# eigenkernel/eigenkernel

Hardware: AMD Instinct MI355X
Metric: eigenpairs/s (full spectrum) + achieved fp64 TFLOP/s vs roofline, N=16384 GEP (higher is better)
Workload: dtype f64

## Files before the change

eigenkernel_amd/csrc/ek_chol.hip:

```cpp
#include "ek_common.h"
#include "ek_block64.h"

#include <cstdlib>
#include <vector>

namespace ek {
namespace {

constexpr int NB = kDiagNB;
constexpr size_t kDiagLds = 2 * b64::IMG * sizeof(double);

__global__ __launch_bounds__(256) void potrf_diag_kernel(int nb, double *B, int ldb, double *inv, int *info,
                                                         int info_base) {
  using namespace b64;
  extern __shared__ double smem[];
  double *sP = smem, *sQ = smem + IMG;
  __shared__ double s_scr[kScratch];
  const int t = threadIdx.x, lane = t & 63, wave = t >> 6, l15 = lane & 15, l4 = lane >> 4;
  auto upper = [&](int gr, int gc) -> double {
    if (gc < nb) return B[(size_t)gc + (size_t)gr * ldb];
    return (gr == gc) ? 1.0 : 0.0;
  };
  auto fail_exit = [&](int j) {
    if (t == 0) atomicCAS(info, 0, info_base + j + 1);
    for (int idx = t; idx < NB * NB; idx += 256)
      inv[idx] = ((idx & (NB - 1)) == (idx >> 7)) ? 1.0 : 0.0;
  };
  for (int idx = t; idx < SB * SB; idx += 256) {
    const int c = idx & 63, r = idx >> 6;
    sP[r * LD + c] = (c >= r) ? upper(r, c) : 0.0;
  }
  __syncthreads();
  int fail = chol64_upper_wg(sP, s_scr);
  if (fail >= 0) { fail_exit(fail); return; }
// ... 197 lines not shown
                 double *work) {
  set_attrs();
  if (n <= 0) return;
  potrf_rec(s, n, B, ldb, 0, invdiag, d_info, work);
}

void trtri256_blocks(hipStream_t s, int n, const double *L, int ldl, const double *invdiag, double *inv256, double *scratch) {
  const int nb2 = n / (2 * NB);
  if (nb2 <= 0) return;
  GemmDesc g{};
  g.M = NB; g.N = NB; g.K = NB; g.transA = false; g.transB = false; g.alpha = 1.0; g.beta = 0.0; g.batch = nb2; g.lower_only = false;
  g.A = L + NB; g.lda = ldl; g.strideA = (long long)2 * NB * ((long long)ldl + 1);
  g.B = invdiag; g.ldb = NB; g.strideB = (long long)2 * NB * NB;
  g.C = scratch; g.ldc = NB; g.strideC = (long long)NB * NB;
  gemm(s, g);
  g.alpha = -1.0;
  g.A = invdiag + (size_t)NB * NB; g.lda = NB; g.strideA = (long long)2 * NB * NB;
  g.B = scratch; g.ldb = NB; g.strideB = (long long)NB * NB;
  g.C = inv256 + NB; g.ldc = 2 * NB; g.strideC = (long long)4 * NB * NB;
  gemm(s, g);
  hipLaunchKernelGGL(inv256_assemble_kernel, dim3(nb2), dim3(256), 0, s, invdiag, inv256);
}
void trsm_register_inv256(const double *invdiag, const double *inv256, int n) {
  g_inv256.base128 = inv256 ? invdiag : nullptr; g_inv256.inv256 = inv256; g_inv256.nblk256 = inv256 ? n / (2 * NB) : 0;
}

void trtri_diag_blocks(hipStream_t s, int n, const double *L, int ldl, double *invdiag) {
  set_attrs();
  if (n <= 0) return;
  hipLaunchKernelGGL(trtri_diag_kernel, dim3(ceil_div(n, NB)), dim3(256),
                     (NB * NB + NB) * sizeof(double), s, n, L, ldl, invdiag);
}


void trsm_rlt(hipStream_t s, int m, int n, const double *L, int ldl, const double *invdiag,
              double *X, int ldx, double *work) {
  if (m <= 0 || n <= 0) return;
  if (const double *i2 = leaf256(invdiag, n)) {
    gemm(s, false, true, m, n, n, 1.0, X, ldx, i2, 2 * NB, 0.0, work, m);
    copy_matrix(s, m, n, work, m, X, ldx);
    return;
  }
  if (n <= NB) {
    gemm(s, false, true, m, n, n, 1.0, X, ldx, invdiag, NB, 0.0, work, m);
    copy_matrix(s, m, n, work, m, X, ldx);
    return;
  }
  const int n1 = split_t(n), n2 = n - n1;
  double *X2 = X + (size_t)n1 * ldx;
  const double *L21 = L + n1, *L22 = L + (size_t)n1 + (size_t)n1 * ldl;
  trsm_rlt(s, m, n1, L, ldl, invdiag, X, ldx, work);
  gemm(s, false, true, m, n2, n1, -1.0, X, ldx, L21, ldl, 1.0, X2, ldx);
  trsm_rlt(s, m, n2, L22, ldl, invdiag + (size_t)(n1 / NB) * NB * NB, X2, ldx, work);
}

void trsm_lln(hipStream_t s, int n, int m, const double *L, int ldl, const double *invdiag,
              double *X, int ldx, double *work) {
  if (m <= 0 || n <= 0) return;
  if (const double *i2 = leaf256(invdiag, n)) {
    gemm(s, false, false, n, m, n, 1.0, i2, 2 * NB, X, ldx, 0.0, work, n);
    copy_matrix(s, n, m, work, n, X, ldx);
    return;
  }
  if (n <= NB) {
    gemm(s, false, false, n, m, n, 1.0, invdiag, NB, X, ldx, 0.0, work, n);
    copy_matrix(s, n, m, work, n, X, ldx);
    return;
  }
  const int n1 = split_t(n), n2 = n - n1;
  double *X2 = X + n1;
  const double *L21 = L + n1, *L22 = L + (size_t)n1 + (size_t)n1 * ldl;
  trsm_lln(s, n1, m, L, ldl, invdiag, X, ldx, work);
  gemm(s, false, false, n2, m, n1, -1.0, L21, ldl, X, ldx, 1.0, X2, ldx);
  trsm_lln(s, n2, m, L22, ldl, invdiag + (size_t)(n1 / NB) * NB * NB, X2, ldx, work);
}

void trsm_llt(hipStream_t s, int n, int m, const double *L, int ldl, const double *invdiag,
              double *X, int ldx, double *work) {
  if (m <= 0 || n <= 0) return;
  if (const double *i2 = leaf256(invdiag, n)) {
    gemm(s, true, false, n, m, n, 1.0, i2, 2 * NB, X, ldx, 0.0, work, n);
    copy_matrix(s, n, m, work, n, X, ldx);
    return;
  }
  if (n <= NB) {
    gemm(s, true, false, n, m, n, 1.0, invdiag, NB, X, ldx, 0.0, work, n);
    copy_matrix(s, n, m, work, n, X, ldx);
    return;
  }
  const int n1 = split_t(n), n2 = n - n1;
  double *X2 = X + n1;
  const double *L21 = L + n1, *L22 = L + (size_t)n1 + (size_t)n1 * ldl;
  trsm_llt(s, n2, m, L22, ldl, invdiag + (size_t)(n1 / NB) * NB * NB, X2, ldx, work);
  gemm(s, true, false, n1, m, n2, -1.0, L21, ldl, X2, ldx, 1.0, X, ldx);
  trsm_llt(s, n1, m, L, ldl, invdiag, X, ldx, work);
}

__global__ void axpy_matrix_kernel(int m, int n, double alpha, const double *__restrict__ src, int lds,
                                   double *__restrict__ dst, int ldd) {
  const int i = blockIdx.x * blockDim.x + threadIdx.x;
  if (i >= m) return;
  for (int j = blockIdx.y; j < n; j += gridDim.y)
    dst[(size_t)i + (size_t)j * ldd] += alpha * src[(size_t)i + (size_t)j * lds];
}
__global__ void full_from_lower_kernel(int n, const double *__restrict__ src, int lds,
                                       double *__restrict__ dst, int ldd) {
  const int i = blockIdx.x * blockDim.x + threadIdx.x;
  if (i >= n) return;
  for (int j = blockIdx.y; j < n; j += gridDim.y)
    dst[(size_t)i + (size_t)j * ldd] = (i >= j) ? src[(size_t)i + (size_t)j * lds] : src[(size_t)j + (size_t)i * lds];
}
__global__ __launch_bounds__(256) void syr2k_fold_kernel(int n, const double *__restrict__ M, int ldm,
                                                         double *__restrict__ A, int lda) {
  __shared__ double sT[32][33];
  const int bi = blockIdx.x, bj = blockIdx.y;
  if (bj > bi) return;
  const int tx = threadIdx.x & 31, ty = threadIdx.x >> 5;
#pragma unroll
  for (int q = 0; q < 4; ++q) {
    const int r = 32 * bj + tx, c = 32 * bi + ty + 8 * q;
// ... 394 lines not shown

void potrf_lower_rl(hipStream_t s, hipStream_t s2, int n, double *B, int ldb, double *invdiag, int *d_info,
                    void *work) {
  set_attrs();
  if (n <= 0) return;
  const PotrfDistLayout Ly(n, ldb, 1);
  const int NRB = Ly.NRB;
  char *w = (char *)work;
  double *ppan = (double *)(w + Ly.off_pbuf);
  int *infos = (int *)(w + Ly.off_infos);
  double *infod = (double *)(w + Ly.off_infod);
  long long *offs = (long long *)(w + Ly.off_offs);
  int *dims = (int *)(w + Ly.off_dims);
  static hipEvent_t evU[2], evP[2], evFork;
  static bool ev_ready = false;
  if (!ev_ready) {
    for (int i = 0; i < 2; ++i) {
      (void)hipEventCreateWithFlags(&evU[i], hipEventDisableTiming);
      (void)hipEventCreateWithFlags(&evP[i], hipEventDisableTiming);
    }
    (void)hipEventCreateWithFlags(&evFork, hipEventDisableTiming);
    ev_ready = true;
  }
  (void)hipMemsetAsync(infos, 0, (size_t)NRB * sizeof(int), s);
  hipLaunchKernelGGL(potrf_table_kernel, dim3(NRB), dim3(round_up(Ly.maxb, 64)), 0, s, n, ldb, 1, 0, NRB, Ly.maxb,
                     offs, dims);
  auto factor_panel = [&](hipStream_t st, int k) {
    const int off = k * NB, nbk = (n - off < NB) ? n - off : NB, mrows = n - off - nbk;
    double *Bd = B + (size_t)off + (size_t)off * ldb;
    double *inv = invdiag + (size_t)k * NB * NB;
    hipLaunchKernelGGL(potrf_diag_kernel, dim3(1), dim3(256), kDiagLds, st, nbk, Bd,
                       ldb, inv, infos + k, off);
    if (mrows > 0) {
      gemm(st, false, true, mrows, nbk, nbk, 1.0, Bd + nbk, ldb, inv, NB, 0.0, ppan, mrows);
      copy_matrix(st, mrows, nbk, ppan, mrows, Bd + nbk, ldb);
    }
  };
  constexpr int ob = 4;
  const int NOB = ceil_div(NRB, ob);
  auto factor_outer = [&](hipStream_t st, int o) {
    const int k0 = o * ob, k1 = (k0 + ob < NRB) ? k0 + ob : NRB;
    for (int k = k0; k < k1; ++k) {
      factor_panel(st, k);
      const int cnt = k1 - 1 - k;
      if (cnt > 0) {
        const int nbk = (n - k * NB < NB) ? n - k * NB : NB;
        GemmDesc g{};
        g.N = NB; g.K = nbk; g.transA = false; g.transB = true; g.alpha = -1.0; g.beta = 1.0;
        g.A = B; g.lda = ldb; g.B = B; g.ldb = ldb; g.C = B; g.ldc = ldb; g.lower_only = true;
        g.even_offs = true;
        g.M = n - (k + 1) * NB; g.batch = cnt;
        g.d_offs = offs + (size_t)k * Ly.maxb * 3; g.d_dims = dims + (size_t)k * Ly.maxb * 3;
        gemm(st, g);
      }
    }
  };
  (void)hipEventRecord(evFork, s);
  (void)hipStreamWaitEvent(s2, evFork, 0);
  factor_outer(s2, 0);
  (void)hipEventRecord(evP[0], s2);
  for (int o = 0; o + 1 < NOB; ++o) {
    const int c0 = o * ob * NB, c1 = (o + 1) * ob * NB, kw = c1 - c0;
    const int m2 = n - c1;
    const int wnext = (m2 < ob * NB) ? m2 : ob * NB;
    (void)hipStreamWaitEvent(s, evP[o & 1], 0);
    const double *P = B + (size_t)c1 + (size_t)c0 * ldb;
    double *C = B + (size_t)c1 + (size_t)c1 * ldb;
    gemm(s, false, true, m2, wnext, kw, -1.0, P, ldb, P, ldb, 1.0, C, ldb, true);
// ... 60 lines not shown
```

eigenkernel_amd/csrc/ek_common.h:

```cpp
#pragma once
#include <hip/hip_runtime.h>
#include <cstddef>
#include <cstdint>
#include <cstdio>

#define EK_HIP_CHECK(expr)                                                              \
  do {                                                                                  \
    hipError_t _e = (expr);                                                             \
    if (_e != hipSuccess) {                                                             \
      fprintf(stderr, "[ek_hip] %s failed at %s:%d: %s\n", #expr, __FILE__, __LINE__,   \
              hipGetErrorString(_e));                                                   \
      return -1000 - (int)_e;                                                           \
    }                                                                                   \
  } while (0)

namespace ek {

constexpr int kWave = 64;

inline int ceil_div(int a, int b) { return (a + b - 1) / b; }
inline int round_up(int a, int b) { return ceil_div(a, b) * b; }

struct GemmDesc {
  int M, N, K;
// ... 43 lines not shown
void set_matrix(hipStream_t s, int m, int n, double offdiag, double diag, double *A, int lda);
void symmetrize_lower(hipStream_t s, int n, double *A, int lda);
void transpose_rows(hipStream_t s, int n, int m, const double *src, int lds, int r0, double *dst, int ldd);
void gather_columns(hipStream_t s, int m, int n, const double *src, int lds, const int *perm,
                    double *dst, int ldd);

void gather_block_cyclic(hipStream_t s, int mr, int nc, const double *src, int lds, int nb, int pr,
                         int me_r, int pc, int me_c, double *dst, int ldd);

void scatter_block_cyclic(hipStream_t s, int mr, int nc, const double *src, int lds, int nb, int pr,
                          int me_r, int pc, int me_c, double *dst, int ldd);

void maxabs_lower(hipStream_t s, int n, const double *A, int lda, double *partial , int bw = 1 << 30);
void scale_lower(hipStream_t s, int n, double alpha, double *A, int lda);
void scale_vector(hipStream_t s, int n, double alpha, double *x);

constexpr int kDiagNB = 128;
void potrf_lower(hipStream_t s, int n, double *B, int ldb, double *invdiag, int *d_info,
                 double *work );
void trtri_diag_blocks(hipStream_t s, int n, const double *L, int ldl, double *invdiag);
void trsm_rlt(hipStream_t s, int m, int n, const double *L, int ldl, const double *invdiag,
              double *X, int ldx, double *work);
void trsm_lln(hipStream_t s, int n, int m, const double *L, int ldl, const double *invdiag,
              double *X, int ldx, double *work);
void trsm_llt(hipStream_t s, int n, int m, const double *L, int ldl, const double *invdiag,
              double *X, int ldx, double *work);
inline size_t sygst_scratch_doubles(int n) {
  const size_t h = (size_t)(n / 2 + 128);
  const size_t a = 2 * h * h, b = 2 * 128 * 128;
  return a > b ? a : b;
}
void trtri256_blocks(hipStream_t s, int n, const double *L, int ldl, const double *invdiag, double *inv256, double *scratch);
void trsm_register_inv256(const double *invdiag, const double *inv256, int n);
void sygst_lower(hipStream_t s, int n, double *A, int lda, const double *L, int ldl,
                 const double *invdiag, double *work, double *scratch);
int sygst_set_direct(int order);
void sygst_scratch_need(int n, size_t need[2]);
int trmm_block_ld(int n);
size_t trmm_diag_doubles(int n);
void trmm_diag_blocks(hipStream_t s, int n, const double *L, int ldl, double *diag);
void trmm_rln(hipStream_t s, int m, int n, const double *L, int ldl, const double *diag, int ldd,
              double *X, int ldx, double *work);
void trmm_llt(hipStream_t s, int n, int m, const double *L, int ldl, const double *diag, int ldd,
              double *X, int ldx, double *work);
void trmm_lln(hipStream_t s, int n, int m, const double *L, int ldl, const double *diag, int ldd,
              double *X, int ldx, double *work);
void sygst2_lower(hipStream_t s, int n, double *A, int lda, const double *L, int ldl, const double *diag,
                  double *work, double *scratch);
struct SygstMember {
  double *A; int lda; const double *L; int ldl; const double *invdiag;
  double *work;
  double *scratch;
  int rank;
};
size_t potrf_rl_work_bytes(int n, int ld);
void potrf_lower_rl(hipStream_t s, hipStream_t s2, int n, double *B, int ldb, double *invdiag, int *d_info,
                    void *work);
struct SytrdExchange;
struct PotrfMember { double *B; int ldb; double *invdiag; int *d_info; void *work; int rank; };
size_t potrf_dist_work_bytes(int n, int ld, int nranks);
void potrf_lower_dist(hipStream_t s, hipStream_t s2, int n, int nmem, const PotrfMember *mem, const SytrdExchange &x);
void potrf_dist_set_lookahead(int on);
void potrf_dist_profile(bool on);
void potrf_dist_profile_collect(double *seconds, int P);
size_t sygst_dist_scratch_doubles(int n, int ld, int nranks);
void sygst_lower_dist(hipStream_t s, int n, int nmem, const SygstMember *mem, const SytrdExchange &x);
// ... 111 lines not shown
```

eigenkernel_amd/csrc/ek_debug.hip:

```cpp
#include "ek_api_internal.h"

using namespace ek;
using namespace ek::api;

extern "C" {

int ek_hip_potrf_team(int n, double *B_loc, const int desc_B[9], int nteam, long long *mismatch) {
  if (n < 0) return -1;
  if (!B_loc && n > 0) return -2;
  int rc = check_desc(desc_B, 3, n, n); if (rc) return rc;
  if (nteam < 0 || nteam > kMaxTeam) return -4;
  rc = ensure_init(); if (rc) return rc;
  if (mismatch) *mismatch = 0;
  if (n == 0) return 0;
  std::lock_guard<std::mutex> lk(g_mu);
  if (nteam == 0 && !g_comm.on) return -4;
  hipStream_t s = g_ctx.stream;
  const int ld = pad_ld(n), nblk = ceil_div(n, kDiagNB);
  const int nmem = nteam > 0 ? nteam : 1, P = nteam > 0 ? nteam : g_comm.nranks;
  const size_t wb = potrf_dist_work_bytes(n, ld, P);
  const size_t per = al((size_t)ld * ld * 8) + al((size_t)nblk * kDiagNB * kDiagNB * 8) + al(wb) + 256;
  void *ws;
  rc = workspace(per * nmem + 256, &ws);
  if (rc) return rc;
// ... 790 lines not shown
  const int old_cols = sytrd_get_max_cols();
  sytrd_set_max_cols(max_cols);
  for (int r = 0; r < reps; ++r) {
    EK_HIP_CHECK(hipMemsetAsync(dA, 0, (size_t)ld * ld * 8, s));
    synth_matrix(s, n, 1, dA, ld);
    EK_HIP_CHECK(hipEventRecord(e0, s));
    sytrd_lower(s, n, dA, ld, vecs, vecs + ld, vecs + 2 * (size_t)ld, nullptr, 0, work);
    EK_HIP_CHECK(hipEventRecord(e1, s));
  }
  sytrd_set_max_cols(old_cols);
  EK_HIP_CHECK(hipStreamSynchronize(s));
  float ms = 0.f; EK_HIP_CHECK(hipEventElapsedTime(&ms, e0, e1));
  (void)hipEventDestroy(e0); (void)hipEventDestroy(e1);
  if (seconds) *seconds = ms * 1e-3;
  return 0;
}

int ek_hip_debug_gemm_at(int transa, int transb, int m, int n, int k, const double *dA, int lda, const double *dB,
                         int ldb, double beta, double *dC, int ldc, int lower_only, int reps, double *seconds) {
  if (m < 1 || n < 1 || k < 1 || !dA || !dB || !dC) return -1;
  int rc = ensure_init(); if (rc) return rc;
  std::lock_guard<std::mutex> lk(g_mu);
  hipStream_t s = g_ctx.stream;
  hipEvent_t e0, e1;
  EK_HIP_CHECK(hipEventCreate(&e0)); EK_HIP_CHECK(hipEventCreate(&e1));
  gemm(s, transa != 0, transb != 0, m, n, k, -1.0, dA, lda, dB, ldb, beta, dC, ldc, lower_only != 0);
  EK_HIP_CHECK(hipEventRecord(e0, s));
  for (int r = 0; r < reps; ++r) gemm(s, transa != 0, transb != 0, m, n, k, -1.0, dA, lda, dB, ldb, beta, dC, ldc, lower_only != 0);
  EK_HIP_CHECK(hipEventRecord(e1, s));
  EK_HIP_CHECK(hipStreamSynchronize(s));
  float ms = 0.f; EK_HIP_CHECK(hipEventElapsedTime(&ms, e0, e1));
  (void)hipEventDestroy(e0); (void)hipEventDestroy(e1);
  if (seconds) *seconds = ms * 1e-3 / (reps > 0 ? reps : 1);
  return 0;
}

}

static int gemm_desc_of(int transa, int transb, int m, int n, int k, double alpha, double beta, const double *dA, int lda,
                        long long strideA, const double *dB, int ldb, long long strideB, double *dC, int ldc,
                        long long strideC, int batch, int lower_only, int staged_rank_k, int small_tiles, int even_offs,
                        const long long *offs, const int *dims, const int *variant, GemmDesc *g) {
  if (transa != 0 && transa != 1) return -1;
  if (transb != 0 && transb != 1) return -2;
  if (m < 0) return -3;
  if (n < 0) return -4;
  if (k < 0) return -5;
  const bool work = m > 0 && n > 0 && batch > 0;
  if (work && k > 0 && !dA) return -8;
  if (lda < 1 || lda < (transa ? k : m)) return -9;
  if (work && k > 0 && !dB) return -11;
  if (ldb < 1 || ldb < (transb ? n : k)) return -12;
  if (work && !dC) return -14;
  if (ldc < 1 || ldc < m) return -15;
  if (batch < 0) return -17;
  if (lower_only != 0 && lower_only != 1) return -18;
  if (staged_rank_k != 0 && staged_rank_k != 1) return -19;
  if (small_tiles != 0 && small_tiles != 1) return -20;
  if (even_offs != 0 && even_offs != 1) return -21;
  if (offs)
    for (int i = 0; i < 3 * batch; ++i) {
      if (offs[i] < 0) return -22;
      if (even_offs && i % 3 != 2 && (offs[i] & 1)) return -21;
    }
  if (dims)
    for (int i = 0; i < 3 * batch; ++i)
// ... 85 lines not shown
```

eigenkernel_amd/solver.py:

```python
import ctypes
import os
from dataclasses import dataclass, field

import numpy as np

from . import descriptor as _d

_HERE = os.path.dirname(os.path.abspath(__file__))
LIB_PATH = os.environ.get("EK_HIP_LIB") or os.path.join(_HERE, "csrc", "libek_hip.so")

N_STAGES = 8
SOLVERS = ("hip", "hip_select", "general_hip", "general_hip_select")
REPLACES = {"hip": "scalapack", "hip_select": "scalapack_select",
            "general_hip": "general_scalapack", "general_hip_select": "general_scalapack_select"}


class LibraryMissing(RuntimeError):
    pass


_lib = None
_dp = ctypes.POINTER(ctypes.c_double)
_ip = ctypes.POINTER(ctypes.c_int)
_llp = ctypes.POINTER(ctypes.c_longlong)
# ... 36 lines not shown
        "ek_hip_sygst_team": (c_int, [c_int, _dp, _ip, _dp, _ip, c_int]),
        "ek_hip_potrf_team": (c_int, [c_int, _dp, _ip, c_int, _llp]),
        "ek_hip_comm_unique_id": (c_int, [vp, c_int]),
        "ek_hip_comm_init": (c_int, [vp, c_int, c_int, c_int]),
        "ek_hip_comm_attach_host": (c_int, [c_int, c_int]),
        "ek_hip_comm_size": (c_int, []),
        "ek_hip_comm_rank": (c_int, []),
        "ek_hip_comm_destroy": (c_int, []),
        "ek_hip_comm_allreduce_device": (c_int, [vp, ctypes.c_longlong]),
        "ek_hip_stedc": (c_int, [c_int, _dp, _dp, _dp, _ip]),
        "ek_hip_ormtr": (c_int, [c_int, c_int, _dp, _ip, _dp, _dp, _ip]),
        "ek_hip_trtrs": (c_int, [c_int, c_int, _dp, _ip, _dp, _ip]),
        "ek_hip_dgemm": (c_int, [c_int, c_int, c_int, c_int, c_int, c_dbl, _dp, c_int, _dp, c_int,
                                 c_dbl, _dp, c_int, c_int]),
        "ek_hip_malloc": (c_int, [ctypes.POINTER(vp), c_ull]),
        "ek_hip_free": (c_int, [vp]),
        "ek_hip_memcpy_h2d": (c_int, [vp, vp, c_ull]),
        "ek_hip_memcpy_d2h": (c_int, [vp, vp, c_ull]),
        "ek_hip_synchronize": (c_int, []),
        "ek_hip_synth_matrix_device": (c_int, [c_int, c_ull, vp, c_int]),
        "ek_hip_residual_device": (c_int, [c_int, c_int, c_int, vp, c_int, vp, c_int, vp, vp, c_int, _dp, _dp, _dp]),
        "ek_hip_orthogonality_device": (c_int, [c_int, c_int, c_int, c_int, vp, c_int, vp, c_int, _dp]),
        "ek_hip_ipratios_device": (c_int, [c_int, c_int, c_int, vp, c_int, vp, c_int, _dp]),
        "ek_hip_check": (c_int, [c_int, c_int, c_int, c_int, c_int, c_int, _dp, _ip, _dp, _ip, _dp, _dp, _ip, _dp]),
        "ek_hip_profile_symv": (c_int, [c_int]),
        "ek_hip_debug_sytrd": (c_int, [c_int, c_int, c_int, _dp]),
        "ek_hip_debug_sytrd_team": (c_int, [c_int, c_int, c_int, _dp]),
        "ek_hip_debug_set_sytrd_maxcols": (c_int, [c_int]),
        "ek_hip_debug_sytrd_work_bytes": (ctypes.c_ulonglong, [c_int]),
        "ek_hip_debug_sytrd_split": (c_int, [vp, c_int]),
        "ek_hip_debug_gemm_at": (c_int, [c_int, c_int, c_int, c_int, c_int, vp, c_int, vp, c_int, c_dbl, vp, c_int,
                                         c_int, c_int, _dp]),
        "ek_hip_debug_sytrd_at": (c_int, [c_int, c_int, c_int, vp, vp, vp, _dp]),
        "ek_hip_debug_gemm_desc": (c_int, [c_int] * 5 + [c_dbl, c_dbl, vp, c_int, c_ll, vp, c_int, c_ll, vp, c_int, c_ll]
                                   + [c_int] * 5 + [_llp, _ip, _ip]),
        "ek_hip_debug_gemm_plan": (c_int, [c_int] * 5 + [c_dbl, c_dbl, vp, c_int, c_ll, vp, c_int, c_ll, vp, c_int, c_ll]
                                   + [c_int] * 5 + [_llp, _ip, _ip]),
        "ek_hip_debug_gemm_compact_map": (c_int, [c_int, c_int, c_ll, c_int, _ip, _ip, _ip]),
        "ek_hip_debug_reduce_team": (c_int, [c_int, c_int, c_int, _dp]),
        "ek_hip_profile_symv_get": (c_int, [_dp, ctypes.POINTER(ctypes.c_longlong), _dp]),
        "ek_hip_debug_sy2sb": (c_int, [c_int, _dp, c_int, _dp, c_int, _dp, _ip]),
        "ek_hip_debug_sy2sb_stage": (c_int, [c_int, _dp, c_int, _dp, c_int, _dp, c_int, _ip]),
        "ek_hip_debug_set_sy2sb_flow": (c_int, [c_int, c_int]),
        "ek_hip_debug_sb2st": (c_int, [c_int, _dp, c_int, _dp, _dp, _dp, c_int, c_int, _ip]),
        "ek_hip_debug_sb2st_stage": (c_int, [c_int, _dp, c_int, c_int, c_int, _dp, _dp, _dp, c_int, _dp, c_int, _dp, c_int,
                                             c_int, _ip, _ip]),
        "ek_hip_debug_two_stage_timing": (c_int, [c_int, c_int, c_int, _dp, _ip]),
        "ek_hip_debug_set_two_stage": (c_int, [c_int]),
        "ek_hip_profile_kernels": (c_int, [c_int]),
        "ek_hip_profile_kernels_get": (c_int, [_dp, _llp]),
        "ek_hip_debug_last_solve_stats": (c_int, [_dp, c_int]),
        "ek_hip_debug_sy2sb_team": (c_int, [c_int, _dp, c_int, _dp, c_int, _dp, c_int, _ip, _llp]),
        "ek_hip_debug_sy2sb_team_timing": (c_int, [c_int, c_int, c_int, _dp]),
        "ek_hip_debug_sy2sb_team_profile": (c_int, [c_int, c_int, c_int, c_int, _dp, _dp]),
        "ek_hip_debug_fail_next_chase": (c_int, [c_int]),
        "ek_hip_debug_stedc_team": (c_int, [c_int, c_int, c_int]),
        "ek_hip_debug_potrf_team_profile": (c_int, [c_int, c_int]),
        "ek_hip_debug_potrf_team_profile_get": (c_int, [c_int, _dp]),
        "ek_hip_debug_stedc_team_get": (c_int, [_dp]),
        "ek_hip_debug_stedc": (c_int, [c_int, _dp, _dp, c_int, c_int, c_int, c_int, c_int, _dp, _dp, c_int, _ip, c_int,
                                       _ip]),
        "ek_hip_debug_stedc_zcols": (c_int, [c_int, c_int]),
        "ek_hip_debug_ormtr": (c_int, [c_int, c_int, _dp, c_int, _dp, _dp, c_int, c_int, c_int]),
        "ek_hip_debug_last_pipe_stats": (c_int, [_dp, c_int]),
        "ek_hip_debug_workspace_bytes": (ctypes.c_ulonglong, [c_int, c_int, c_int, c_int, ctypes.POINTER(ctypes.c_ulonglong)]),
        "ek_hip_eigenvalues_device": (c_int, [c_int, c_int, c_int, c_int, vp, c_int, vp, c_int, vp, _dp, c_int]),
# ... 124 lines not shown
                                               c_int, c_int, c_int, c_int, _dp, _dp]),
        "ek_hip_check_sparse": (c_int, [c_int, c_int, c_ll, _ip, _dp, c_ll, _ip, _dp, _dp, _dp, c_int,
                                        c_int, c_int, c_int, c_int, _dp, _dp]),
        "ek_hip_sparse_to_dense": (c_int, [c_int, c_ll, _ip, _dp, _dp, c_int]),
        "ek_hip_debug_sparse_check_workspace_bytes": (c_ull, [c_int, c_int, c_ll, c_ll, c_int, c_int, c_int, c_int]),
        "ek_hip_debug_sparse_csr": (c_ll, [c_int, c_ll, _ip, _dp, _llp, _ip, _dp]),
    }
    for name, (res, args) in sigs.items():
        try:
            fn = getattr(lib, name)
        except AttributeError:
            if os.environ.get("EK_HIP_BRINGUP") == "1":
                continue
            raise
        fn.restype = res
        fn.argtypes = args
    if path is None:
        _lib = lib
    return lib


EXPORTED_SYMBOLS = (
    "ek_hip_version", "ek_hip_init", "ek_hip_finalize", "ek_hip_stage_name", "ek_hip_solve",
    "ek_hip_solve_device", "ek_hip_solve_replicated", "ek_hip_solve_device_grid",
    "ek_hip_set_allgatherv", "ek_hip_gather_matrix", "ek_hip_potrf", "ek_hip_sygst", "ek_hip_sytrd", "ek_hip_stedc",
    "ek_hip_ormtr", "ek_hip_trtrs", "ek_hip_dgemm", "ek_hip_malloc", "ek_hip_free",
    "ek_hip_memcpy_h2d", "ek_hip_memcpy_d2h", "ek_hip_synchronize", "ek_hip_synth_matrix_device",
    "ek_hip_profile_symv", "ek_hip_profile_symv_get", "ek_hip_debug_sytrd",
    "ek_hip_residual_device", "ek_hip_orthogonality_device", "ek_hip_ipratios_device", "ek_hip_check",
    "ek_hip_sytrd_team", "ek_hip_comm_unique_id", "ek_hip_comm_init", "ek_hip_comm_size", "ek_hip_comm_rank",
    "ek_hip_comm_destroy", "ek_hip_comm_allreduce_device", "ek_hip_debug_sytrd_team", "ek_hip_sygst_team",
    "ek_hip_potrf_team", "ek_hip_debug_reduce_team", "ek_hip_comm_attach_host",
    "ek_hip_debug_set_sytrd_maxcols", "ek_hip_debug_sytrd_work_bytes", "ek_hip_debug_sytrd_at", "ek_hip_debug_sytrd_split", "ek_hip_debug_gemm_at",
    "ek_hip_debug_gemm_desc", "ek_hip_debug_gemm_plan", "ek_hip_debug_gemm_compact_map",
    "ek_hip_debug_sy2sb", "ek_hip_debug_sy2sb_stage", "ek_hip_debug_set_sy2sb_flow", "ek_hip_debug_sb2st", "ek_hip_debug_sb2st_stage", "ek_hip_debug_two_stage_timing", "ek_hip_debug_set_two_stage",
    "ek_hip_profile_kernels", "ek_hip_profile_kernels_get", "ek_hip_debug_last_solve_stats",
    "ek_hip_debug_sy2sb_team", "ek_hip_debug_sy2sb_team_timing", "ek_hip_debug_sy2sb_team_profile", "ek_hip_debug_workspace_bytes", "ek_hip_debug_fail_next_chase", "ek_hip_debug_last_pipe_stats",
    "ek_hip_debug_stedc_team", "ek_hip_debug_stedc_team_get", "ek_hip_debug_stedc",
    "ek_hip_debug_stedc_zcols", "ek_hip_debug_ormtr",
    "ek_hip_debug_potrf_team_profile", "ek_hip_debug_potrf_team_profile_get",
    "ek_hip_eigenvalues_device", "ek_hip_eigenvalues", "ek_hip_stebz",
    "ek_hip_debug_values_workspace_bytes", "ek_hip_debug_set_stebz",
    "ek_hip_eigenpairs_device", "ek_hip_eigenpairs", "ek_hip_stebz_range", "ek_hip_debug_window_workspace_bytes",
    "ek_hip_sygvx_device", "ek_hip_sygvx", "ek_hip_sygst_ibtype", "ek_hip_trmm", "ek_hip_debug_sygvx_workspace_bytes",
    "ek_hip_eigenpairs_batched_device", "ek_hip_eigenpairs_batched",
    "ek_hip_eigenpairs_vbatched_device", "ek_hip_eigenpairs_vbatched",
    "ek_hip_debug_vbatched_streams", "ek_hip_debug_vbatched_last",
    "ek_hip_check_batched_device", "ek_hip_check_batched", "ek_hip_check_vbatched_device", "ek_hip_check_vbatched",
    "ek_hip_sygv_batched_device", "ek_hip_sygv_batched", "ek_hip_sygv_vbatched_device", "ek_hip_sygv_vbatched",
    "ek_hip_check_sygv_batched_device", "ek_hip_check_sygv_batched", "ek_hip_check_sygv_vbatched_device",
    "ek_hip_check_sygv_vbatched", "ek_hip_check_sygvx_device", "ek_hip_check_sygvx",
    "ek_hip_eigenpairs_xbatched_device", "ek_hip_eigenpairs_xbatched", "ek_hip_debug_xbatched_chunk",
    "ek_hip_check_xbatched_device", "ek_hip_check_xbatched", "ek_hip_debug_check_xbatched_chunk",
    "ek_hip_sygv_xbatched_device", "ek_hip_sygv_xbatched",
    "ek_hip_check_sygv_xbatched_device", "ek_hip_check_sygv_xbatched",
    "ek_hip_eigenpairs_xvbatched_device", "ek_hip_eigenpairs_xvbatched", "ek_hip_sygv_xvbatched_device",
    "ek_hip_sygv_xvbatched", "ek_hip_debug_xvbatched_last",
    "ek_hip_eigenpairs_window_xvbatched_device", "ek_hip_eigenpairs_window_xvbatched",
    "ek_hip_sygv_window_xvbatched_device", "ek_hip_sygv_window_xvbatched", "ek_hip_debug_window_xvbatched_budget",
    "ek_hip_check_xvbatched_device", "ek_hip_check_xvbatched", "ek_hip_check_sygv_xvbatched_device",
    "ek_hip_check_sygv_xvbatched", "ek_hip_debug_check_xvbatched_last",
    "ek_hip_debug_stage_leaves256", "ek_hip_debug_set_sygst_direct", "ek_hip_debug_sygst_scratch",
    "ek_hip_solve_sparse", "ek_hip_check_sparse_device", "ek_hip_check_sparse", "ek_hip_sparse_to_dense",
    "ek_hip_debug_sparse_check_workspace_bytes", "ek_hip_debug_sparse_csr",
    "ek_hip_eigenpairs_window_batched_device", "ek_hip_eigenpairs_window_batched", "ek_hip_debug_window_batched_chunk",
    "ek_hip_eigenpairs_window_xbatched_device", "ek_hip_eigenpairs_window_xbatched",
# ... 1250 lines not shown
```

include/ek_hip_debug.h:

```cpp
#ifndef EK_HIP_DEBUG_H
#define EK_HIP_DEBUG_H

#ifdef __cplusplus
extern "C" {
#endif

int ek_hip_profile_symv(int enable);
int ek_hip_profile_symv_get(double *seconds, long long *launches, double *algorithmic_bytes);

int ek_hip_profile_kernels(int enable);
int ek_hip_profile_kernels_get(double *seconds , long long *launches );

int ek_hip_debug_sytrd(int n, int ld, int reps, double *seconds);
unsigned long long ek_hip_debug_sytrd_work_bytes(int n);
int ek_hip_debug_sytrd_at(int n, int max_cols, int reps, double *dA, void *work, double *vecs, double *seconds);
int ek_hip_debug_gemm_at(int transa, int transb, int m, int n, int k, const double *dA, int lda, const double *dB,
                         int ldb, double beta, double *dC, int ldc, int lower_only, int reps, double *seconds);
int ek_hip_debug_gemm_desc(int transa, int transb, int m, int n, int k, double alpha, double beta, const double *dA, int lda,
                           long long strideA, const double *dB, int ldb, long long strideB, double *dC, int ldc,
                           long long strideC, int batch, int lower_only, int staged_rank_k, int small_tiles, int even_offs,
                           const long long *offs, const int *dims, int *variant );
int ek_hip_debug_gemm_plan(int transa, int transb, int m, int n, int k, double alpha, double beta, const double *dA, int lda,
                           long long strideA, const double *dB, int ldb, long long strideB, double *dC, int ldc,
                           long long strideC, int batch, int lower_only, int staged_rank_k, int small_tiles, int even_offs,
                           const long long *offs, const int *dims, int *variant );
int ek_hip_debug_gemm_compact_map(int tiles_m, int tiles_n, long long first, int count, int *tm, int *tn, int *valid);
int ek_hip_debug_sytrd_split(void *alt, int mask);
int ek_hip_debug_set_sytrd_maxcols(int max_cols);
int ek_hip_debug_sytrd_team(int n, int nteam, int reps, double *seconds);
int ek_hip_debug_reduce_team(int n, int nteam, int reps, double *seconds );

int ek_hip_debug_sy2sb(int n, double *A, int lda, double *V, int ldv, double *tau, int *flag);
int ek_hip_debug_sb2st(int n, const double *A, int lda, double *d, double *e, double *Z, int ldz, int ncols, int *flag);
int ek_hip_debug_two_stage_timing(int n, int ncols, int reps, double *seconds, int *flag);
int ek_hip_debug_set_two_stage(int min_order);
int ek_hip_debug_sy2sb_stage(int n, double *A, int lda, double *V, int ldv, double *tau, int poison, int *flag);
int ek_hip_debug_set_sy2sb_flow(int pair_min, int lookahead_min);
int ek_hip_debug_sb2st_stage(int n, const double *A, int lda, int form, int chase_mode, double *d, double *e, double *V2,
                             int ldv2, double *tau2, int ldtau, double *Z, int ldz, int ncols, int *ran, int *flag);
int ek_hip_debug_sy2sb_team(int n, double *A, int lda, double *V, int ldv, double *tau, int nteam, int *flag,
                            long long *mismatch);
int ek_hip_debug_sy2sb_team_timing(int n, int nteam, int reps, double *seconds);
int ek_hip_debug_sy2sb_team_profile(int n, int nteam, int reps, int lookahead_min, double *seconds, double *parts);

int ek_hip_debug_last_solve_stats(double *out, int count);

unsigned long long ek_hip_debug_workspace_bytes(int problem, int n, int n_vec, int nranks, unsigned long long *parts);

unsigned long long ek_hip_debug_values_workspace_bytes(int problem, int n);
int ek_hip_debug_set_stebz(int lanes);
unsigned long long ek_hip_debug_window_workspace_bytes(int problem, int n, int jobz, int range, int m);
unsigned long long ek_hip_debug_sygvx_workspace_bytes(int itype, int n, int jobz, int range, int m);
unsigned long long ek_hip_debug_sparse_check_workspace_bytes(int problem, int n, long long nnzA, long long nnzB,
                                                             int n_check, int index1, int index2, int n_ipr);
long long ek_hip_debug_sparse_csr(int n, long long nnz, const int *suf, const double *val, long long *rowptr, int *col,
                                  double *csr_val);
int ek_hip_debug_vbatched_streams(int streams);
int ek_hip_debug_vbatched_last(double *class_seconds, int *class_count);
int ek_hip_debug_xvbatched_last(double *class_seconds, int *class_count);
// ... 33 lines not shown
```

Before: 20490.

## Add in-place MFMA TRSM leaf kernel replacing GEMM plus copy

Adds a dedicated leaf kernel that multiplies a strip of X by the 128 or 256 inverted diagonal block using f64 MFMA and writes the result back in place. It replaces the generic GEMM into a workspace followed by copy_matrix in the trsm leaves and in the Cholesky panel solve. This removes an extra pass over memory and a kernel launch per leaf. The price is a specialised kernel with a strip-width heuristic, alignment checks on the inverse pointer, and possibly lower throughput than the tuned GEMM for large free dimensions.

```diff
diff --git a/eigenkernel_amd/csrc/ek_chol.hip b/eigenkernel_amd/csrc/ek_chol.hip
--- a/eigenkernel_amd/csrc/ek_chol.hip
+++ b/eigenkernel_amd/csrc/ek_chol.hip
@@ -1,5 +1,6 @@
 #include "ek_common.h"
 #include "ek_block64.h"
+#include "ek_trsm_leaf.h"
 
 #include <cstdlib>
 #include <vector>
@@ -263,18 +264,45 @@
                      (NB * NB + NB) * sizeof(double), s, n, L, ldl, invdiag);
 }
 
+static bool leaf_has_kernel(int n, const double *inv) { return (n == NB || n == 2 * NB) && ((uintptr_t)inv & 31) == 0; }
+static void leaf_launch(hipStream_t s, int form, int n, int free, const double *inv, double *X, int ldx, int W) {
+  if (form == leaf::kLeafLeftN) leaf::launch_leaf_n<leaf::kLeafLeftN>(s, n, free, inv, X, ldx, W);
+  else if (form == leaf::kLeafLeftT) leaf::launch_leaf_n<leaf::kLeafLeftT>(s, n, free, inv, X, ldx, W);
+  else leaf::launch_leaf_n<leaf::kLeafRightT>(s, n, free, inv, X, ldx, W);
+}
+static bool trsm_leaf(hipStream_t s, int form, int n, int free, const double *inv, double *X, int ldx) {
+  if (free <= 0 || !leaf_has_kernel(n, inv)) return false;
+  leaf_launch(s, form, n, free, inv, X, ldx, leaf::strip_width(n, free));
+  return true;
+}
+static void trsm_leaf_gemm(hipStream_t s, int form, int n, int free, const double *inv, int ldi, double *X, int ldx,
+                           double *work) {
+  if (form == leaf::kLeafRightT) {
+    gemm(s, false, true, free, n, n, 1.0, X, ldx, inv, ldi, 0.0, work, free);
+    copy_matrix(s, free, n, work, free, X, ldx);
+  } else {
+    gemm(s, form == leaf::kLeafLeftT, false, n, free, n, 1.0, inv, ldi, X, ldx, 0.0, work, n);
+    copy_matrix(s, n, free, work, n, X, ldx);
+  }
+}
+int trsm_leaf_debug(hipStream_t s, int form, int n, int free, const double *inv, double *X, int ldx, double *work, int path) {
+  const bool kernel = form >= 0 && form <= 2 && leaf_has_kernel(n, inv);
+  if (path != 0 && path != 2 && !kernel) return -1;
+  if (path == 0 || !kernel) { trsm_leaf_gemm(s, form, n, free, inv, n, X, ldx, work); return 0; }
+  leaf_launch(s, form, n, free, inv, X, ldx, path == 3 ? leaf::kNarrow : path == 4 ? leaf::kWide : leaf::strip_width(n, free));
+  return 1;
+}
+
 
 void trsm_rlt(hipStream_t s, int m, int n, const double *L, int ldl, const double *invdiag,
               double *X, int ldx, double *work) {
   if (m <= 0 || n <= 0) return;
   if (const double *i2 = leaf256(invdiag, n)) {
-    gemm(s, false, true, m, n, n, 1.0, X, ldx, i2, 2 * NB, 0.0, work, m);
-    copy_matrix(s, m, n, work, m, X, ldx);
+    if (!trsm_leaf(s, leaf::kLeafRightT, n, m, i2, X, ldx)) trsm_leaf_gemm(s, leaf::kLeafRightT, n, m, i2, 2 * NB, X, ldx, work);
     return;
   }
   if (n <= NB) {
-    gemm(s, false, true, m, n, n, 1.0, X, ldx, invdiag, NB, 0.0, work, m);
-    copy_matrix(s, m, n, work, m, X, ldx);
+    if (!trsm_leaf(s, leaf::kLeafRightT, n, m, invdiag, X, ldx)) trsm_leaf_gemm(s, leaf::kLeafRightT, n, m, invdiag, NB, X, ldx, work);
     return;
   }
   const int n1 = split_t(n), n2 = n - n1;
@@ -289,13 +317,11 @@
               double *X, int ldx, double *work) {
   if (m <= 0 || n <= 0) return;
   if (const double *i2 = leaf256(invdiag, n)) {
-    gemm(s, false, false, n, m, n, 1.0, i2, 2 * NB, X, ldx, 0.0, work, n);
-    copy_matrix(s, n, m, work, n, X, ldx);
+    if (!trsm_leaf(s, leaf::kLeafLeftN, n, m, i2, X, ldx)) trsm_leaf_gemm(s, leaf::kLeafLeftN, n, m, i2, 2 * NB, X, ldx, work);
     return;
   }
   if (n <= NB) {
-    gemm(s, false, false, n, m, n, 1.0, invdiag, NB, X, ldx, 0.0, work, n);
-    copy_matrix(s, n, m, work, n, X, ldx);
+    if (!trsm_leaf(s, leaf::kLeafLeftN, n, m, invdiag, X, ldx)) trsm_leaf_gemm(s, leaf::kLeafLeftN, n, m, invdiag, NB, X, ldx, work);
     return;
   }
   const int n1 = split_t(n), n2 = n - n1;
@@ -310,13 +336,11 @@
               double *X, int ldx, double *work) {
   if (m <= 0 || n <= 0) return;
   if (const double *i2 = leaf256(invdiag, n)) {
-    gemm(s, true, false, n, m, n, 1.0, i2, 2 * NB, X, ldx, 0.0, work, n);
-    copy_matrix(s, n, m, work, n, X, ldx);
+    if (!trsm_leaf(s, leaf::kLeafLeftT, n, m, i2, X, ldx)) trsm_leaf_gemm(s, leaf::kLeafLeftT, n, m, i2, 2 * NB, X, ldx, work);
     return;
   }
   if (n <= NB) {
-    gemm(s, true, false, n, m, n, 1.0, invdiag, NB, X, ldx, 0.0, work, n);
-    copy_matrix(s, n, m, work, n, X, ldx);
+    if (!trsm_leaf(s, leaf::kLeafLeftT, n, m, invdiag, X, ldx)) trsm_leaf_gemm(s, leaf::kLeafLeftT, n, m, invdiag, NB, X, ldx, work);
     return;
   }
   const int n1 = split_t(n), n2 = n - n1;
@@ -777,8 +801,10 @@
     hipLaunchKernelGGL(potrf_diag_kernel, dim3(1), dim3(256), kDiagLds, st, nbk, Bd,
                        ldb, inv, infos + k, off);
     if (mrows > 0) {
-      gemm(st, false, true, mrows, nbk, nbk, 1.0, Bd + nbk, ldb, inv, NB, 0.0, ppan, mrows);
-      copy_matrix(st, mrows, nbk, ppan, mrows, Bd + nbk, ldb);
+      if (!trsm_leaf(st, leaf::kLeafRightT, nbk, mrows, inv, Bd + nbk, ldb)) {
+        gemm(st, false, true, mrows, nbk, nbk, 1.0, Bd + nbk, ldb, inv, NB, 0.0, ppan, mrows);
+        copy_matrix(st, mrows, nbk, ppan, mrows, Bd + nbk, ldb);
+      }
     }
   };
   constexpr int ob = 4;
diff --git a/eigenkernel_amd/csrc/ek_common.h b/eigenkernel_amd/csrc/ek_common.h
--- a/eigenkernel_amd/csrc/ek_common.h
+++ b/eigenkernel_amd/csrc/ek_common.h
@@ -99,6 +99,7 @@
 }
 void trtri256_blocks(hipStream_t s, int n, const double *L, int ldl, const double *invdiag, double *inv256, double *scratch);
 void trsm_register_inv256(const double *invdiag, const double *inv256, int n);
+int trsm_leaf_debug(hipStream_t s, int form, int n, int free, const double *inv, double *X, int ldx, double *work, int path);
 void sygst_lower(hipStream_t s, int n, double *A, int lda, const double *L, int ldl,
                  const double *invdiag, double *work, double *scratch);
 int sygst_set_direct(int order);
diff --git a/eigenkernel_amd/csrc/ek_debug.hip b/eigenkernel_amd/csrc/ek_debug.hip
--- a/eigenkernel_amd/csrc/ek_debug.hip
+++ b/eigenkernel_amd/csrc/ek_debug.hip
@@ -846,6 +846,42 @@
   float ms = 0.f; EK_HIP_CHECK(hipEventElapsedTime(&ms, e0, e1));
   (void)hipEventDestroy(e0); (void)hipEventDestroy(e1);
   if (seconds) *seconds = ms * 1e-3 / (reps > 0 ? reps : 1);
+  return 0;
+}
+
+int ek_hip_debug_trsm_leaf(int form, int n, int free, const double *dInv, double *dX, int ldx, double *dWork, int path,
+                           int reps, double *seconds, int *taken) {
+  if (form < 0 || form > 2) return -1;
+  if (n < 1) return -2;
+  if (free < 1) return -3;
+  if (!dInv) return -4;
+  if (!dX) return -5;
+  if (ldx < (form == 2 ? free : n)) return -6;
+  if (path < 0 || path > 4) return -8;
+  const bool kernel_only = path == 1 || path >= 3;
+  if (kernel_only && n != kDiagNB && n != 2 * kDiagNB) return -8;
+  if (!dWork && !kernel_only) return -7;
+  if (reps < 0) return -9;
+  int rc = ensure_init(); if (rc) return rc;
+  std::lock_guard<std::mutex> lk(g_mu);
+  hipStream_t s = g_ctx.stream;
+  if (kernel_only && ((uintptr_t)dInv & 31)) return -4;
+  int ran = trsm_leaf_debug(s, form, n, free, dInv, dX, ldx, dWork, path);
+  EK_HIP_CHECK(hipGetLastError());
+  EK_HIP_CHECK(hipStreamSynchronize(s));
+  if (taken) *taken = ran;
+  if (reps > 0) {
+    hipEvent_t e0, e1;
+    EK_HIP_CHECK(hipEventCreate(&e0)); EK_HIP_CHECK(hipEventCreate(&e1));
+    EK_HIP_CHECK(hipEventRecord(e0, s));
+    for (int r = 0; r < reps; ++r) trsm_leaf_debug(s, form, n, free, dInv, dX, ldx, dWork, path);
+    EK_HIP_CHECK(hipEventRecord(e1, s));
+    EK_HIP_CHECK(hipGetLastError());
+    EK_HIP_CHECK(hipStreamSynchronize(s));
+    float ms = 0.f; EK_HIP_CHECK(hipEventElapsedTime(&ms, e0, e1));
+    (void)hipEventDestroy(e0); (void)hipEventDestroy(e1);
+    if (seconds) *seconds = ms * 1e-3 / reps;
+  }
   return 0;
 }
 
diff --git a/eigenkernel_amd/csrc/ek_trsm_leaf.h b/eigenkernel_amd/csrc/ek_trsm_leaf.h
--- /dev/null
+++ b/eigenkernel_amd/csrc/ek_trsm_leaf.h
@@ -0,0 +1,177 @@
+#pragma once
+
+#ifndef EK_LEAF_HD
+#if defined(__HIPCC__)
+#define EK_LEAF_HD __host__ __device__
+#else
+#define EK_LEAF_HD
+#endif
+#endif
+
+namespace ek {
+namespace leaf {
+
+enum Form { kLeafLeftN = 0, kLeafLeftT = 1, kLeafRightT = 2 };
+
+constexpr int kWide = 32, kNarrow = 16;
+
+EK_LEAF_HD inline int wide_min_strips(int n) { return n > 128 ? 256 : 512; }
+EK_LEAF_HD inline int strip_width(int n, int free) {
+  return (free + kWide - 1) / kWide >= wide_min_strips(n) ? kWide : kNarrow;
+}
+EK_LEAF_HD inline int strip_count(int free, int W) { return free > 0 ? (free + W - 1) / W : 0; }
+EK_LEAF_HD inline int strip_first(int wg, int W) { return wg * W; }
+EK_LEAF_HD inline int strip_valid(int free, int W, int wg) {
+  const int left = free - wg * W;
+  return left <= 0 ? 0 : (left < W ? left : W);
+}
+EK_LEAF_HD inline long long elem_offset(int form, int a, int f, int ldx) {
+  return form == kLeafRightT ? (long long)f + (long long)a * ldx : (long long)a + (long long)f * ldx;
+}
+EK_LEAF_HD inline int strip_ld(int n) { return n + 2; }
+EK_LEAF_HD inline unsigned long long strip_lds_bytes(int n, int W) { return (unsigned long long)W * strip_ld(n) * 8ull; }
+
+}
+}
+
+#if defined(__HIPCC__)
+namespace ek {
+namespace leaf {
+
+typedef double leaf_double4_t __attribute__((ext_vector_type(4)));
+
+template <bool HALVES>
+__device__ __forceinline__ void swap_rows(double &a, double &b) {
+  typedef unsigned leaf_uint2_t __attribute__((ext_vector_type(2)));
+  const unsigned alo = (unsigned)__double2loint(a), ahi = (unsigned)__double2hiint(a);
+  const unsigned blo = (unsigned)__double2loint(b), bhi = (unsigned)__double2hiint(b);
+  const leaf_uint2_t lo = HALVES ? __builtin_amdgcn_permlane32_swap(alo, blo, false, false)
+                                 : __builtin_amdgcn_permlane16_swap(alo, blo, false, false);
+  const leaf_uint2_t hi = HALVES ? __builtin_amdgcn_permlane32_swap(ahi, bhi, false, false)
+                                 : __builtin_amdgcn_permlane16_swap(ahi, bhi, false, false);
+  a = __hiloint2double((int)hi.x, (int)lo.x);
+  b = __hiloint2double((int)hi.y, (int)lo.y);
+}
+
+template <int FORM, int N, int W>
+__global__ __launch_bounds__(256, 2) void trsm_leaf_kernel(int free, const double *__restrict__ inv, double *X, int ldx) {
+  extern __shared__ double s_strip[];
+  constexpr int LDK = N + 2;
+  constexpr bool LEFT = FORM != kLeafRightT;
+  constexpr int AI = N / 64, FI = W / 16;
+  constexpr int KB = 4;
+  const int t = threadIdx.x, lane = t & 63, wave = t >> 6, l15 = lane & 15, l4 = lane >> 4;
+  const int f0 = strip_first(blockIdx.x, W), cnt = strip_valid(free, W, blockIdx.x);
+  if (cnt <= 0) return;
+
+  constexpr int PER = N * W / 256;
+#pragma unroll
+  for (int i0 = 0; i0 < PER; i0 += 8) {
+    double r[8];
+#pragma unroll
+    for (int i = 0; i < 8; ++i) {
+      const int idx = t + 256 * (i0 + i);
+      const int k = LEFT ? idx % N : idx / W, f = LEFT ? idx / N : idx % W;
+      r[i] = f < cnt ? X[LEFT ? (size_t)k + (size_t)(f0 + f) * ldx : (size_t)(f0 + f) + (size_t)k * ldx] : 0.0;
+    }
+#pragma unroll
+    for (int i = 0; i < 8; ++i) {
+      const int idx = t + 256 * (i0 + i);
+      const int k = LEFT ? idx % N : idx / W, f = LEFT ? idx / N : idx % W;
+      s_strip[f * LDK + k] = r[i];
+    }
+  }
+
+  const int aw = wave * (N / 4);
+  static_assert(KB == 4, "a batch is one 32-byte piece per lane and a 4 x 4 exchange");
+  auto fetch = [&](leaf_double4_t (&raw)[AI], int kk) {
+#pragma unroll
+    for (int ai = 0; ai < AI; ++ai) {
+      const int a = aw + 16 * ai + l15;
+      if (FORM == kLeafLeftT) {
+        raw[ai] = *reinterpret_cast<const leaf_double4_t *>(inv + (size_t)(kk + 4 * l4) + (size_t)a * N);
+      } else {
+#pragma unroll
+        for (int q = 0; q < KB; ++q) raw[ai][q] = inv[(size_t)a + (size_t)(kk + 4 * q + l4) * N];
+      }
+    }
+  };
+  auto unpack = [&](const leaf_double4_t (&raw)[AI], double (&g)[KB][AI]) {
+#pragma unroll
+    for (int ai = 0; ai < AI; ++ai) {
+      if (FORM == kLeafLeftT) {
+        double v0 = raw[ai][0], v1 = raw[ai][1], v2 = raw[ai][2], v3 = raw[ai][3];
+        swap_rows<true>(v0, v2); swap_rows<true>(v1, v3);
+        swap_rows<false>(v0, v1); swap_rows<false>(v2, v3);
+        g[0][ai] = v0; g[1][ai] = v1; g[2][ai] = v2; g[3][ai] = v3;
+      } else {
+#pragma unroll
+        for (int q = 0; q < KB; ++q) g[q][ai] = raw[ai][q];
+      }
+    }
+  };
+  leaf_double4_t raw[AI];
+  double g[KB][AI];
+  fetch(raw, 0);
+
+  leaf_double4_t acc[FI][AI];
+#pragma unroll
+  for (int fi = 0; fi < FI; ++fi)
+#pragma unroll
+    for (int ai = 0; ai < AI; ++ai) acc[fi][ai] = (leaf_double4_t){0.0, 0.0, 0.0, 0.0};
+
+  __syncthreads();
+
+  for (int kk = 0; kk < N; kk += 4 * KB) {
+    unpack(raw, g);
+    if (kk + 4 * KB < N) fetch(raw, kk + 4 * KB);
+#pragma unroll
+    for (int q = 0; q < KB; ++q) {
+      double x[FI];
+#pragma unroll
+      for (int fi = 0; fi < FI; ++fi) x[fi] = s_strip[(16 * fi + l15) * LDK + kk + 4 * q + l4];
+#pragma unroll
+      for (int fi = 0; fi < FI; ++fi)
+#pragma unroll
+        for (int ai = 0; ai < AI; ++ai)
+          acc[fi][ai] = LEFT ? __builtin_amdgcn_mfma_f64_16x16x4f64(x[fi], g[q][ai], acc[fi][ai], 0, 0, 0)
+                             : __builtin_amdgcn_mfma_f64_16x16x4f64(g[q][ai], x[fi], acc[fi][ai], 0, 0, 0);
+    }
+  }
+
+#pragma unroll
+  for (int fi = 0; fi < FI; ++fi)
+#pragma unroll
+    for (int ai = 0; ai < AI; ++ai)
+#pragma unroll
+      for (int r = 0; r < 4; ++r) {
+        const int a = aw + 16 * ai + (LEFT ? l15 : l4 + 4 * r);
+        const int f = 16 * fi + (LEFT ? l4 + 4 * r : l15);
+        if (f < cnt) X[LEFT ? (size_t)a + (size_t)(f0 + f) * ldx : (size_t)(f0 + f) + (size_t)a * ldx] = acc[fi][ai][r];
+      }
+}
+
+template <int FORM, int N, int W>
+inline void launch_leaf(hipStream_t s, int free, const double *inv, double *X, int ldx) {
+  static bool attr_set = false;
+  const size_t lds = (size_t)strip_lds_bytes(N, W);
+  if (!attr_set) {
+    (void)hipFuncSetAttribute((const void *)trsm_leaf_kernel<FORM, N, W>, hipFuncAttributeMaxDynamicSharedMemorySize, (int)lds);
+    attr_set = true;
+  }
+  hipLaunchKernelGGL((trsm_leaf_kernel<FORM, N, W>), dim3(strip_count(free, W)), dim3(256), lds, s, free, inv, X, ldx);
+}
+template <int FORM>
+inline void launch_leaf_n(hipStream_t s, int n, int free, const double *inv, double *X, int ldx, int W) {
+  if (n == 256) {
+    if (W == kWide) launch_leaf<FORM, 256, kWide>(s, free, inv, X, ldx);
+    else launch_leaf<FORM, 256, kNarrow>(s, free, inv, X, ldx);
+  } else {
+    if (W == kWide) launch_leaf<FORM, 128, kWide>(s, free, inv, X, ldx);
+    else launch_leaf<FORM, 128, kNarrow>(s, free, inv, X, ldx);
+  }
+}
+
+}
+}
+#endif
diff --git a/eigenkernel_amd/solver.py b/eigenkernel_amd/solver.py
--- a/eigenkernel_amd/solver.py
+++ b/eigenkernel_amd/solver.py
@@ -92,6 +92,7 @@
         "ek_hip_debug_gemm_at": (c_int, [c_int, c_int, c_int, c_int, c_int, vp, c_int, vp, c_int, c_dbl, vp, c_int,
                                          c_int, c_int, _dp]),
         "ek_hip_debug_sytrd_at": (c_int, [c_int, c_int, c_int, vp, vp, vp, _dp]),
+        "ek_hip_debug_trsm_leaf": (c_int, [c_int, c_int, c_int, vp, vp, c_int, vp, c_int, c_int, _dp, _ip]),
         "ek_hip_debug_gemm_desc": (c_int, [c_int] * 5 + [c_dbl, c_dbl, vp, c_int, c_ll, vp, c_int, c_ll, vp, c_int, c_ll]
                                    + [c_int] * 5 + [_llp, _ip, _ip]),
         "ek_hip_debug_gemm_plan": (c_int, [c_int] * 5 + [c_dbl, c_dbl, vp, c_int, c_ll, vp, c_int, c_ll, vp, c_int, c_ll]
@@ -282,6 +283,7 @@
     "ek_hip_comm_destroy", "ek_hip_comm_allreduce_device", "ek_hip_debug_sytrd_team", "ek_hip_sygst_team",
     "ek_hip_potrf_team", "ek_hip_debug_reduce_team", "ek_hip_comm_attach_host",
     "ek_hip_debug_set_sytrd_maxcols", "ek_hip_debug_sytrd_work_bytes", "ek_hip_debug_sytrd_at", "ek_hip_debug_sytrd_split", "ek_hip_debug_gemm_at",
+    "ek_hip_debug_trsm_leaf",
     "ek_hip_debug_gemm_desc", "ek_hip_debug_gemm_plan", "ek_hip_debug_gemm_compact_map",
     "ek_hip_debug_sy2sb", "ek_hip_debug_sy2sb_stage", "ek_hip_debug_set_sy2sb_flow", "ek_hip_debug_sb2st", "ek_hip_debug_sb2st_stage", "ek_hip_debug_two_stage_timing", "ek_hip_debug_set_two_stage",
     "ek_hip_profile_kernels", "ek_hip_profile_kernels_get", "ek_hip_debug_last_solve_stats",
diff --git a/include/ek_hip_debug.h b/include/ek_hip_debug.h
--- a/include/ek_hip_debug.h
+++ b/include/ek_hip_debug.h
@@ -25,6 +25,8 @@
                            long long strideC, int batch, int lower_only, int staged_rank_k, int small_tiles, int even_offs,
                            const long long *offs, const int *dims, int *variant );
 int ek_hip_debug_gemm_compact_map(int tiles_m, int tiles_n, long long first, int count, int *tm, int *tn, int *valid);
+int ek_hip_debug_trsm_leaf(int form, int n, int free, const double *dInv, double *dX, int ldx, double *dWork, int path,
+                           int reps, double *seconds, int *taken);
 int ek_hip_debug_sytrd_split(void *alt, int mask);
 int ek_hip_debug_set_sytrd_maxcols(int max_cols);
 int ek_hip_debug_sytrd_team(int n, int nteam, int reps, double *seconds);
```

Result: no change. 20570, median of 6 (+0.4%).
